# mbhall88/nohuman

Measured on AMD Instinct MI355X. Metric: Mreads/sec classified (HPRC.r2 DB, 150bp PE), higher is better.
Workload: dtype u64

## Files before the change

### nohuman_amd/csrc/nh_device.h

```cpp
#pragma once
#include <stdint.h>

namespace nh {

struct DevDB {
    const uint32_t *table;
    uint64_t copy_stride;
    uint32_t n_copies;
    uint32_t copy_shift;
    uint64_t capacity;
    uint64_t cap_magic;
    const uint32_t *parent;
    uint32_t node_count;
    uint32_t value_bits;
    uint32_t vmask;
    uint32_t k, l;
    uint32_t window;
    uint64_t lmer_mask;
    uint64_t spaced_mask;
    uint64_t toggle;
    uint64_t min_hash;
    int32_t revcom_version;
    int32_t linear_probing;
    int32_t reset_per_mate;
    uint32_t min_hit_groups;
    int32_t ambig_rule;
    uint32_t max_chunks;
};

enum { CNT_FRAGMENTS = 0, CNT_CLASSIFIED = 1, CNT_BASES = 2, CNT_LOOKUPS = 3, CNT_N = 4 };

struct Result {
    uint32_t call, total_kmers, clade_hits, hit_groups;
};

struct Sched {
    uint64_t n0, n01, total;
    uint64_t base1, base2;
    uint32_t c0, c1, c2, pad;
};

constexpr uint32_t TAIL_SHARDS = 8;
constexpr uint32_t WORK_WORDS = 1 + TAIL_SHARDS;
constexpr uint32_t WORK_STRIDE = 16;
constexpr uint32_t WORK_PASSES = 3;
constexpr uint32_t COUNTER_SHARDS = 64;
constexpr uint32_t COUNTER_STRIDE = 16;

constexpr uint32_t SEG_TILES = 32;
constexpr uint32_t SPLIT_MIN_TILES = 48;
constexpr uint32_t MID_TILES = 8;
constexpr uint32_t PART_DWORDS = 64;
constexpr uint32_t PART_CAP = 30;
struct SplitItem {
    uint32_t f, seg, nseg, slot;
};
struct SplitHdr {
    uint32_t n_multi, n_mid, n_small, seg_used;
};
struct SplitBufs {
    SplitHdr *hdr;
    SplitItem *items_multi;
    uint32_t *items_single;
    uint32_t *part;
    uint32_t *part_done;
    uint32_t seg_cap, pad;
};

struct KArgs {
    DevDB db;
    const uint8_t *bases;
    const uint64_t *seq_off;
    const uint32_t *seq_len;
    uint64_t bases_end;
    uint64_t n_frag;
    int32_t mates;
    uint32_t frag_chunk;
    Sched sched;
    double confidence;
    Result *out;
    uint32_t *kmer_taxa;
    const uint64_t *kmer_taxa_off;
    unsigned long long *counters;
    unsigned long long *cshard;
    int *error_flag;
    int *pending;
    uint32_t *defer_bits;
    int *pending_long;
    int32_t only_deferred;
    unsigned long long *work;
    SplitBufs split;
    unsigned long long *timeline;
};

struct SchedKnobs {
    bool set = false, off = false;
    uint32_t c1 = 0, c2 = 0, p1 = 100, p2 = 100;
};
struct LaunchIO {
    const void *d_bases = nullptr;
    const void *d_seq_off = nullptr;
    const void *d_seq_len = nullptr;
    uint64_t bases_end = 0;
    uint64_t n_frag = 0;
    int mates = 1;
    bool long_reads = false;
    void *d_out = nullptr, *d_kmer_taxa = nullptr;
    const void *d_kmer_taxa_off = nullptr;
    void *d_counters = nullptr;
};
struct LaunchSlot {
    int *d_error = nullptr;
    int *d_pending = nullptr;
    int *d_pending_long = nullptr;
    unsigned long long *d_work = nullptr;
    unsigned long long *d_cshard = nullptr;
    uint32_t *d_defer = nullptr;
    uint64_t defer_cap_bits = 0;
    SplitBufs split = {};
    uint64_t split_single_cap = 0;
    bool split_fresh = false;
};

constexpr uint32_t TAXON_AMBIGUOUS = 0xFFFFFFFFu;
constexpr uint32_t TAXON_MATE_BORDER = 0xFFFFFFFEu;

constexpr int WAVE = 64;
constexpr int WAVES_PER_BLOCK = 4;
constexpr int TL = 128;
constexpr int LIST_CAP = 64;

}
```

### nohuman_amd/csrc/nh_engine.hip

```cpp
#include <hip/hip_runtime.h>
#include <stdarg.h>
#include <stdio.h>
#include <stdlib.h>
#include <string.h>
#include <sys/stat.h>
#include <algorithm>
#include <thread>
#include <unistd.h>
#include <fcntl.h>

#include <chrono>
#include <mutex>
#include <string>
#include <vector>

#include "nh_device.h"
#include <map>

#include "nh_internal.h"
#include "nohuman_engine.h"

namespace nh {

namespace {
// ... 271 lines not shown
    d.node_count = (uint32_t)i.node_count;
    d.value_bits = (uint32_t)i.value_bits;
    d.vmask = (uint32_t)((1ull << i.value_bits) - 1);
    d.k = (uint32_t)i.k;
    d.l = (uint32_t)i.l;
    d.window = (uint32_t)(i.k - i.l);
    d.lmer_mask = (1ull << (2 * i.l)) - 1;
    d.spaced_mask = i.spaced_seed_mask ? i.spaced_seed_mask : ~0ull;
    d.toggle = i.toggle_mask & d.lmer_mask;
    d.min_hash = i.minimum_acceptable_hash_value;
    d.revcom_version = i.revcom_version;
    d.linear_probing = e->options.linear_probing;
    d.reset_per_mate = e->options.reset_per_mate;
    d.min_hit_groups = e->options.minimum_hit_groups;
    d.ambig_rule = e->options.ambiguity_rule == NH_AMBIGUITY_LAST_LMER ? 0 : 1;
    d.max_chunks = i.capacity + 1 > 0xFFFFFFFFull ? 0xFFFFFFFFu : (uint32_t)(i.capacity + 1);
}

void finish_devdb_public(Engine *e) { finish_devdb(e); }

static int alloc_table(Engine *e, uint64_t capacity) {
    e->table_cells_alloc = ((capacity + 3) & ~3ull) + 32;
    uint32_t want = 4;
    if (const char *env = getenv("NOHUMAN_TABLE_COPIES")) {
        const int v = atoi(env);
        want = v >= 8 ? 8u : v >= 4 ? 4u : v >= 2 ? 2u : 1u;
    }
    {
        const nh_db_info &i = e->info;
        const bool std_geom = i.k == 35 && i.l == 31 && i.revcom_version != 0 && i.minimum_acceptable_hash_value == 0;
        bool quad = std_geom && e->options.linear_probing != 0;
#ifdef NH_NO_QUAD
        quad = false;
#endif
        if (capacity >= 0xFFFFFF00ull && !quad) want = 1;
    }
    bool trimmed = false;
    for (;; want >>= 1) {
        const uint64_t sh = 32 / want;
        const uint64_t stride = ((e->table_cells_alloc + 32 + 31) & ~31ull) - (want > 1 ? sh : 0);
        const size_t bytes = (size_t)(stride * want + 64) * sizeof(uint32_t) + 256;
        hipError_t he = hipMalloc(&e->d_table_raw, bytes);
        if (he != hipSuccess && !trimmed) {
            (void)hipGetLastError();
            run_cache_trim();
            dev_cache_trim();
            (void)dev_set(e->device);
            trimmed = true;
            he = hipMalloc(&e->d_table_raw, bytes);
        }
        if (he == hipSuccess) {
            if (dev_debug()) dev_register(e->d_table_raw, bytes, e->device);
            e->d_table = (uint32_t *)(((uintptr_t)e->d_table_raw + 127) & ~(uintptr_t)127);
            e->n_copies = want;
            e->copy_stride = stride;
            if (getenv("NOHUMAN_TRACE"))
                fprintf(stderr, "[nohuman trace] hash table: %u staggered cop%s of %.2f GB\n", want, want == 1 ? "y" : "ies",
                        (double)e->table_cells_alloc * 4 / 1e9);
            return NH_OK;
        }
        (void)hipGetLastError();
        if (want == 1) return set_error(NH_EOOM, "cannot allocate the hash table (%zu bytes)", bytes);
    }
}

int refresh_table_copies(Engine *e) {
    HIP_TRY(dev_set(e->device));
    HIP_TRY(hipDeviceSynchronize());
    for (uint32_t j = 1; j < e->n_copies; j++)
        HIP_TRY(hipMemcpyAsync(e->d_table + j * e->copy_stride, e->d_table, e->table_cells_alloc * sizeof(uint32_t),
                               hipMemcpyDeviceToDevice, e->stream));
    HIP_TRY(hipStreamSynchronize(e->stream));
    return NH_OK;
}

LaunchKnobs read_launch_knobs() {
    LaunchKnobs kn;
    if (const char *env = getenv("NOHUMAN_FRAG_CHUNK")) kn.frag_chunk = (uint32_t)std::max(1, atoi(env));
    if (const char *env = getenv("NOHUMAN_SEG_CAP")) {
        const long v = atol(env);
        if (v >= 1) kn.seg_cap = (uint64_t)v;
    }
    kn.sched = parse_sched_knobs(getenv("NOHUMAN_SCHED"));
    return kn;
}

static int validate_table(Engine *e, bool check_size) {
    auto t0 = std::chrono::steady_clock::now();
    unsigned long long *d_out = (unsigned long long *)e->d_counters + CNT_N;
    unsigned long long out[2] = {0, 0};
    HIP_TRY(hipMemsetAsync(d_out, 0, sizeof out, e->stream));
    HIP_TRY(launch_validate_table(e->d_table, e->table_cells_alloc & ~3ull, (uint32_t)((1ull << e->info.value_bits) - 1), d_out, e->stream));
    HIP_TRY(hipMemcpyAsync(out, d_out, sizeof out, hipMemcpyDeviceToHost, e->stream));
    HIP_TRY(hipMemsetAsync(d_out, 0, sizeof out, e->stream));
    HIP_TRY(hipStreamSynchronize(e->stream));
    e->check.non_empty = out[0];
    e->check.max_value = out[1];
    e->check.seconds = std::chrono::duration<double>(std::chrono::steady_clock::now() - t0).count();
    if (getenv("NOHUMAN_TRACE"))
        fprintf(stderr, "[nohuman trace] hash table checked in %.4f s: %llu of %llu cells in use (load %.4f), largest value %llu, taxonomy nodes %llu\n",
                e->check.seconds, out[0], (unsigned long long)e->info.capacity, (double)out[0] / (double)e->info.capacity, out[1],
                (unsigned long long)e->info.node_count);
    if (out[1] >= e->info.node_count)
        return set_error(NH_EDB, "hash.k2d holds the taxon value %llu but taxo.k2d has only %llu nodes: the two files are not of one database",
                         out[1], (unsigned long long)e->info.node_count);
    if (check_size && out[0] != e->info.size)
        return set_error(NH_EDB, "hash.k2d: %llu cells are in use but its header says size %llu", out[0], (unsigned long long)e->info.size);
    return NH_OK;
}

static int common_open(Engine *e, int device) {
    int rc = check_device(device);
    if (rc) return rc;
    e->device = device;
    e->info.device = device;
    HIP_TRY(dev_set(device));
    hipDeviceProp_t prop;
    HIP_TRY(hipGetDeviceProperties(&prop, dev_phys(device)));
    e->n_cu = prop.multiProcessorCount;
    e->grid_blocks = e->n_cu * classify_blocks_per_cu();
    e->options.minimum_hit_groups = 2;
    e->options.linear_probing = 1;
    e->options.reset_per_mate = 1;
    e->options.ambiguity_rule = NH_AMBIGUITY_DEFAULT;
    bool overridden = false;
    if (const char *v = getenv("NOHUMAN_OPT_AMBIGUITY_RULE")) e->options.ambiguity_rule = atoi(v) != 0 ? NH_AMBIGUITY_QUEUE : NH_AMBIGUITY_LAST_LMER, overridden = true;
    if (const char *v = getenv("NOHUMAN_OPT_LINEAR_PROBING")) e->options.linear_probing = atoi(v) != 0, overridden = true;
    if (const char *v = getenv("NOHUMAN_OPT_RESET_PER_MATE")) e->options.reset_per_mate = atoi(v) != 0, overridden = true;
    if (const char *v = getenv("NOHUMAN_OPT_MIN_HIT_GROUPS")) e->options.minimum_hit_groups = (uint32_t)atoi(v), overridden = true;
    if (overridden) {
        static std::atomic<bool> said{false};
        if (!said.exchange(true))
            fprintf(stderr, "nohuman: WARN NOHUMAN_OPT_* overrides the classification switches of every engine of this process: ambiguity rule %s, "
                            "linear probing %d, per-mate reset %d, minimum hit groups %u\n",
                    e->options.ambiguity_rule == NH_AMBIGUITY_QUEUE ? "queue" : "last l-mer", e->options.linear_probing, e->options.reset_per_mate,
                    e->options.minimum_hit_groups);
    }
    e->knobs = read_launch_knobs();
    HIP_TRY(hipStreamCreateWithFlags(&e->stream, hipStreamNonBlocking));
    for (unsigned i = 0; i < LAUNCH_SLOTS; i++) HIP_TRY(hipEventCreateWithFlags(&e->slot_ev[i], hipEventDisableTiming));
    HIP_TRY(dev_malloc((void **)&e->d_counters, (CNT_N + 12) * sizeof(uint64_t)));
    HIP_TRY(hipMemset(e->d_counters, 0, (CNT_N + 12) * sizeof(uint64_t)));
    HIP_TRY(dev_malloc((void **)&e->d_work, LAUNCH_SLOTS * WORK_PASSES * WORK_WORDS * WORK_STRIDE * sizeof(unsigned long long)));
    HIP_TRY(hipMemset(e->d_work, 0, LAUNCH_SLOTS * WORK_PASSES * WORK_WORDS * WORK_STRIDE * sizeof(unsigned long long)));
    HIP_TRY(dev_malloc((void **)&e->d_cshard, LAUNCH_SLOTS * COUNTER_SHARDS * COUNTER_STRIDE * sizeof(unsigned long long)));
    HIP_TRY(hipMemset(e->d_cshard, 0, LAUNCH_SLOTS * COUNTER_SHARDS * COUNTER_STRIDE * sizeof(unsigned long long)));
    HIP_TRY(dev_malloc((void **)&e->d_error, (2 * LAUNCH_SLOTS + 1) * sizeof(int)));
    HIP_TRY(hipMemset(e->d_error, 0, (2 * LAUNCH_SLOTS + 1) * sizeof(int)));
    HIP_TRY(dev_malloc((void **)&e->d_defer, LAUNCH_SLOTS * DEFER_WORDS * sizeof(uint32_t)));
    HIP_TRY(hipMemset(e->d_defer, 0, LAUNCH_SLOTS * DEFER_WORDS * sizeof(uint32_t)));
    return NH_OK;
}

static int upload_taxonomy(Engine *e) {
    HIP_TRY(dev_malloc((void **)&e->d_parent, e->parent.size() * sizeof(uint32_t)));
    HIP_TRY(hipMemcpy(e->d_parent, e->parent.data(), e->parent.size() * sizeof(uint32_t),
                      hipMemcpyHostToDevice));
    return NH_OK;
}

void destroy(Engine *e) {
    if (!e) return;
    if (e->device >= 0) (void)dev_set(e->device);
    if (e->d_table_raw) (void)hipFree(e->d_table_raw);
    if (e->d_parent) (void)hipFree(e->d_parent);
    if (e->d_counters) (void)hipFree(e->d_counters);
    if (e->d_error) (void)hipFree(e->d_error);
    if (e->d_external) (void)hipFree(e->d_external);
    if (e->d_work) (void)hipFree(e->d_work);
    if (e->d_cshard) (void)hipFree(e->d_cshard);
    if (e->d_defer) (void)hipFree(e->d_defer);
    for (SplitBufs &sb : e->split)
        for (void *p : {(void *)sb.hdr, (void *)sb.items_multi, (void *)sb.items_single, (void *)sb.part, (void *)sb.part_done})
            if (p) (void)hipFree(p);
    for (void *p : {e->st.d_bases, e->st.d_offsets, e->st.d_results, e->st.d_taxa, e->st.d_taxa_off})
        if (p) (void)hipFree(p);
    for (hipEvent_t ev : e->slot_ev)
        if (ev) (void)hipEventDestroy(ev);
    if (e->stream) (void)hipStreamDestroy(e->stream);
    delete e;
}

int open_images(const void *opts, size_t opts_len, const void *taxo, size_t taxo_len,
                const void *hash, size_t hash_len, int device, Engine **out) {
    if (!opts || !taxo || !hash || !out) return set_error(NH_EINVAL, "null argument");
    Engine *e = new Engine();
    int rc = common_open(e, device);
    if (!rc) rc = parse_opts(e, opts, opts_len);
    if (!rc) rc = parse_taxonomy(e, taxo, taxo_len);
    if (!rc) {
        const uint8_t *hb = (const uint8_t *)hash;
        if (hash_len < 32) rc = set_error(NH_EDB, "hash.k2d: truncated header");
        else {
            e->info.capacity = rd64(hb);
            e->info.size = rd64(hb + 8);
            e->info.key_bits = rd64(hb + 16);
            e->info.value_bits = rd64(hb + 24);
            if (e->info.key_bits + e->info.value_bits != 32 || e->info.value_bits == 0 ||
                e->info.value_bits > 31)
                rc = set_error(NH_EDB, "hash.k2d: key_bits + value_bits != 32");
            else if (e->info.capacity == 0 || hash_len != 32 + 4 * e->info.capacity)
                rc = set_error(NH_EDB, "hash.k2d: size %zu != 32 + 4*capacity (%llu)", hash_len,
                               (unsigned long long)e->info.capacity);
        }
        if (!rc) rc = check_queue_packing(e);
        if (!rc) rc = alloc_table(e, e->info.capacity);
        if (!rc) {
            hipError_t he = hipMemset(e->d_table, 0, e->table_cells_alloc * sizeof(uint32_t));
            if (he == hipSuccess)
                he = hipMemcpy(e->d_table, hb + 32, 4 * e->info.capacity, hipMemcpyHostToDevice);
            if (he != hipSuccess) rc = set_error(NH_EDEVICE, "table upload: %s", hipGetErrorString(he));
        }
    }
    if (!rc) rc = validate_table(e, true);
    if (!rc) rc = upload_taxonomy(e);
    if (!rc) rc = refresh_table_copies(e);
    if (rc) {
        destroy(e);
        return rc;
    }
    finish_devdb(e);
// ... 692 lines not shown
```

### nohuman_amd/csrc/nh_internal.h

```cpp
#pragma once
#include <hip/hip_runtime.h>
#include <stdint.h>

#include <atomic>
#include <mutex>
#include <string>
#include <vector>

#include "nh_device.h"
#include "nohuman_engine.h"

namespace nh {
constexpr unsigned LAUNCH_SLOTS = 16;
constexpr uint64_t DEFER_WORDS = 1u << 15;
}

namespace nh {

struct Staging {
    void *d_bases = nullptr, *d_offsets = nullptr, *d_results = nullptr, *d_taxa = nullptr,
         *d_taxa_off = nullptr;
    size_t cap_bases = 0, cap_offsets = 0, cap_results = 0, cap_taxa = 0, cap_taxa_off = 0;
};

struct LaunchKnobs {
    uint32_t frag_chunk = 0;
    uint64_t seg_cap = 0;
    SchedKnobs sched;
};
LaunchKnobs read_launch_knobs();
SchedKnobs parse_sched_knobs(const char *env);

struct TableCheck {
    uint64_t non_empty = 0, max_value = 0;
    double seconds = 0;
};

struct Engine {
    int device = -1;
    int n_cu = 0;
    int grid_blocks = 0;
    nh_db_info info{};
    nh_options options{};
    DevDB dev{};
    void *d_table_raw = nullptr;
    uint32_t *d_table = nullptr;
    uint32_t n_copies = 1;
    uint64_t copy_stride = 0;
    uint64_t table_cells_alloc = 0;
    uint32_t *d_parent = nullptr;
    uint64_t *d_counters = nullptr;
    int *d_error = nullptr;
    unsigned long long *d_work = nullptr;
    unsigned long long *d_cshard = nullptr;
    uint32_t *d_defer = nullptr;
    SplitBufs split[LAUNCH_SLOTS] = {};
    uint64_t split_single_cap[LAUNCH_SLOTS] = {};
    bool split_fresh[LAUNCH_SLOTS] = {};
    std::mutex split_mu;
    std::atomic<unsigned> launch_seq{0};
    hipEvent_t slot_ev[LAUNCH_SLOTS] = {};
    bool slot_used[LAUNCH_SLOTS] = {};
    std::mutex slot_mu[LAUNCH_SLOTS];
    LaunchKnobs knobs;
    TableCheck check;
    hipStream_t stream = nullptr;
    std::vector<uint32_t> parent;
    std::vector<uint64_t> external;
    uint64_t *d_external = nullptr;
    std::vector<uint8_t> taxo_image, opts_image;
    Staging st;
    std::mutex mu;
    std::mutex db_mu;
    double seconds = 0;
};

extern thread_local std::string g_last_error;
int set_error(int code, const char *fmt, ...) __attribute__((format(printf, 2, 3)));

hipError_t launch_classify(const DevDB &db, const LaunchIO &io, double confidence, const LaunchSlot &sl,
                           uint32_t frag_chunk, int grid_blocks, hipStream_t stream, const SchedKnobs &sched_knobs);
Sched make_sched(uint64_t n_frag, uint32_t c0, int mates, uint64_t waves, const SchedKnobs &kn);
hipError_t launch_validate_table(const uint32_t *table, uint64_t n_cells, uint32_t vmask, unsigned long long *d_out2,
                                 hipStream_t stream);
int classify_blocks_per_cu();
hipError_t launch_insert_sequences(const DevDB &db, const void *d_bases, const void *d_seq_off,
                                   uint64_t n_seq, uint32_t value, unsigned long long *d_inserted,
                                   int grid_blocks, hipStream_t stream);
hipError_t launch_synth_insert(uint32_t *table, uint64_t capacity, uint64_t cap_magic,
                               uint32_t value_bits, uint32_t value, uint64_t n_keys, uint64_t seed,
                               uint64_t key_mask, unsigned long long *d_size, hipStream_t stream);

int open_dir(const char *db_dir, int device, Engine **out);
int open_images(const void *opts, size_t opts_len, const void *taxo, size_t taxo_len,
                const void *hash, size_t hash_len, int device, Engine **out);
int open_synthetic(uint64_t capacity, uint64_t n_keys, uint32_t depth, uint64_t seed, int device,
                   Engine **out);
void destroy(Engine *e);
void finish_devdb_public(Engine *e);
int refresh_table_copies(Engine *e);
int resolve_db_dir(const char *db_dir, std::string &resolved);
int classify_device(Engine *e, const void *d_bases, const void *d_seq_off, uint64_t n_frag,
                    uint32_t flags, double confidence, void *d_results, void *d_kmer_taxa,
                    const void *d_kmer_taxa_off, void *d_counters, hipStream_t stream,
                    const void *d_seq_len = nullptr, uint64_t bases_end = 0);
int classify_host(Engine *e, const uint8_t *bases, const uint64_t *seq_offsets, uint64_t n_frag,
                  uint32_t flags, double confidence, nh_result *results, uint32_t *kmer_taxa,
                  uint64_t *kmer_taxa_offsets, uint64_t kmer_taxa_cap);
int check_error_flag(Engine *e);
struct HumanOutArgs {
    const char *text;
// ... 64 lines not shown
```

### nohuman_amd/csrc/nh_kernels.hip

```cpp
#include <hip/hip_runtime.h>
#include <stdlib.h>
#include <string.h>

#include <type_traits>

#include "nh_device.h"

namespace nh {

#define NH_FULL 0xFFFFFFFFFFFFFFFFull
#ifndef NH_WIDE_CELLS
#define NH_WIDE_CELLS 16
#endif
#ifndef NH_WIDE_AFTER
#define NH_WIDE_AFTER 2
#endif
#ifndef NH_R2_CELLS
#define NH_R2_CELLS 4
#endif

template <bool STD> struct CandPad { static constexpr int value = STD ? 6 : 66; };

#ifndef NH_MIN_WAVES
#define NH_MIN_WAVES 5
// ... 1053 lines not shown
                                      kmer_taxa, kt, prof, tprev);
            if ((flags & 2u) && reset_per_mate) st.carry_tax = 0;
            bool finish = (flags & 1u) != 0;
            if (SPLIT && finish && (flags & 16u)) {
                const uint32_t nseg = uni(d0.y), seg = d_nk0, sb = uni(d1.w);
                KArgsP a4 = launder(ap);
                const bool over = st.overflow || st.nlist > PART_CAP;
                uint32_t v = 0;
                if (lane == 0) v = st.hit_groups;
                if (lane == 1) v = over ? 0u : st.nlist;
                if (lane == 2) v = over ? 1u : 0u;
                if (lane >= 4 && !over) {
                    const uint32_t idx = ((uint32_t)lane - 4u) >> 1;
                    if (idx < st.nlist) {
                        if constexpr (BIG) v = (lane & 1) ? TLI.cnt[idx] : TLI.tax[idx];
                        else v = (lane & 1) ? S.list_cnt[idx] : S.list_tax[idx];
                    }
                }
                __hip_atomic_store(&a4->split.part[(uint64_t)(sb + seg) * PART_DWORDS + (uint32_t)lane], v, __ATOMIC_RELAXED,
                                   __HIP_MEMORY_SCOPE_AGENT);
                asm volatile("s_waitcnt vmcnt(0)" ::: "memory");
                uint32_t old = 0;
                if (lane == 0) old = atomicAdd(&a4->split.part_done[sb], 1u);
                old = uni(old);
                finish = old + 1u == nseg;
                __atomic_signal_fence(__ATOMIC_SEQ_CST);
                if (finish) {
                    for (uint32_t s2 = 0; s2 < nseg; s2++) {
                        if (s2 == seg) continue;
                        const uint32_t pv = __hip_atomic_load(&a4->split.part[(uint64_t)(sb + s2) * PART_DWORDS + (uint32_t)lane],
                                                              __ATOMIC_RELAXED, __HIP_MEMORY_SCOPE_AGENT);
                        st.hit_groups += __builtin_amdgcn_readlane(pv, 0);
                        const uint32_t n2 = __builtin_amdgcn_readlane(pv, 1);
                        if (__builtin_amdgcn_readlane(pv, 2)) st.overflow = true;
                        for (uint32_t i = 0; i < n2; i++)
                            list_add<BIG>(S, TLI, lane, st, __builtin_amdgcn_readlane(pv, 4 + 2 * (int)i),
                                          __builtin_amdgcn_readlane(pv, 5 + 2 * (int)i));
                    }
                    if (over) st.overflow = true;
                }
            }
            if (finish) {
                const uint32_t total_kmers = d_total;
                uint32_t call = 0, clade_hits = 0;
                if (st.nlist > 0) {
                    if (BIG) {
                        call = resolve_tree_big(ap, TLI, lane, st, total_kmers, clade_hits);
                    } else if (st.nlist == 1) {
                        const uint32_t cnt = S.list_cnt[0];
                        const uint32_t required = (uint32_t)ceil(a2->confidence * (double)total_kmers);
                        call = cnt >= required ? S.list_tax[0] : 0u;
                        if (call && st.hit_groups < a2->db.min_hit_groups) call = 0;
                        clade_hits = call ? cnt : 0u;
                    } else {
                        call = resolve_tree<STD>(ap, S, lane, st, total_kmers, clade_hits);
                    }
                }
                const bool defer = !BIG && st.overflow;
                if (defer) call = 0;
                if (lane == 0) {
                    uint4 rec;
                    rec.x = defer ? CALL_OVERFLOW : call;
                    rec.y = total_kmers;
                    rec.z = clade_hits;
                    rec.w = st.hit_groups;
                    const uint32_t sn = S.stage_n;
                    S.stage_rec[sn] = rec;
                    S.stage_f[sn] = f;
                    S.stage_n = sn + 1;
                    if (kmer_taxa && mates == 2)
                        kmer_taxa[a2->kmer_taxa_off[f] + d_nk0] = TAXON_MATE_BORDER;
                    if (defer) atomicMax(&a2->pending[0], 1);
                    if (BIG && st.overflow) atomicOr(&a2->error_flag[0], 1);
                }
                if (lane == 0 && call) S.acc[CNT_CLASSIFIED] += 1;
            }
            wave_sync();
        }
        if (lane == 0) S.frag_state = make_uint4(st.nlist, st.hit_groups, st.carry_tax, st.overflow ? 1u : 0u);
        NH_STAMP(7);
    }

constexpr uint32_t PREF_LANES = 42;
constexpr uint32_t SHORT_MAX = 158;

__device__ __forceinline__ bool sample_all_long(KArgsP ap, const int lane) {
    KArgsP a = launder(ap);
    const uint64_t ns = a->n_frag * (uint64_t)a->mates;
    const uint64_t i = ns * (uint64_t)lane / 64u;
    const uint32_t len = a->seq_len != nullptr ? a->seq_len[i] : (uint32_t)(a->seq_off[i + 1] - a->seq_off[i]);
    return __ballot(len <= SHORT_MAX) == 0;
}

template <bool LINEAR, bool STD, bool CAP32, bool PROF, bool BIG>
__global__ __launch_bounds__(WAVE * WAVES_PER_BLOCK, BIG ? 1 : (STD ? NH_MIN_WAVES : 3)) void k_classify(const KArgs args_by_kernarg_pointer) {
    KArgsP ap = (KArgsP)__builtin_amdgcn_kernarg_segment_ptr();
    if (BIG && ap->pending[0] == 0) return;
    bool only_deferred = ap->only_deferred != 0;
    if (only_deferred && ap->pending_long[0] == 0) {
        if (BIG || !sample_all_long(ap, (int)(threadIdx.x & 63))) return;
        only_deferred = false;
    }
    typedef WaveLdsT<STD, 1, QCAP_GENERIC> WL;
    __shared__ WL lds_all[WAVES_PER_BLOCK];
    __shared__ uint32_t big_lists[BIG ? WAVES_PER_BLOCK * 3 * BIG_LIST_CAP : 1];
    const int lane = threadIdx.x & 63;
    const int wib = __builtin_amdgcn_readfirstlane(threadIdx.x >> 6);
    WL &S = lds_all[wib];
    TaxList TLI = {nullptr, nullptr, nullptr, 0};
    if constexpr (BIG) {
        TLI.tax = &big_lists[(wib * 3 + 0) * BIG_LIST_CAP];
        TLI.cnt = &big_lists[(wib * 3 + 1) * BIG_LIST_CAP];
        TLI.score = &big_lists[(wib * 3 + 2) * BIG_LIST_CAP];
        TLI.cap = BIG_LIST_CAP;
    }

    init_wave_lds<STD>(S, lane);

    const uint32_t K = STD ? 35u : ap->db.k;
    const uint32_t L = STD ? 31u : ap->db.l;
    const uint32_t TQ = TL - (STD ? 4u : ap->db.window);
    const int mates = ap->mates;
    const uint64_t n_frag = ap->n_frag;
    const bool reset_per_mate = ap->db.reset_per_mate != 0;
    const bool inplace = ap->seq_len != nullptr;
    if (lane == 0) S.last_dw = ((inplace ? ap->bases_end : ap->seq_off[n_frag * (uint64_t)mates]) + 4) >> 2;
    const uint32_t pl = (uint32_t)lane < PREF_LANES ? (uint32_t)lane : PREF_LANES - 1;

    auto tile_ptr = [&](uint64_t g0) -> const uint32_t * {
        KArgsP a3 = launder(ap);
        const uint64_t last_dw = S.last_dw;
        uint64_t dw = (g0 >> 2) + pl;
        dw = dw < last_dw ? dw : last_dw;
        return reinterpret_cast<const uint32_t *>(a3->bases) + dw;
    };

    if (lane < 4) S.acc[lane] = 0;
    bool bad_input = false;
    uint64_t prof[12] = {0, 0, 0, 0, 0, 0, 0, 0, 0, 0, 0, 0};
    uint64_t tprev = PROF ? __builtin_readcyclecounter() : 0;

#ifndef NH_PF_DEPTH
#define NH_PF_DEPTH 2
#endif
    constexpr int PFD = NH_PF_DEPTH;
    uint32_t tagf[PFD], wf[PFD];
#pragma unroll
    for (int i = 0; i < PFD; i++) tagf[i] = 0, wf[i] = 0;

    uint32_t par = 0;
    uint32_t nslot_new = 0;
    uint32_t nslot_old = 0;
    uint32_t qn = 0;
    LaneLookup lk;
    lk.busy = 0;
    lk.r = 0;
    lk.pos = lk.first_pos = lk.step = 0;
    lk.ckey = 0;
    lk.budget = 0;

    if (lane == 0) S.frag_state = make_uint4(0, 0, 0, 0);
    uint64_t carry_pack = 0;
    auto turn = [&]() {
        flush_records<STD>(ap, S, lane);
#ifndef NH_NO_QUAD
        if constexpr (LINEAR && STD)
// ... 202 lines not shown
                        d1.y = qn;
                        d1.z = nruns;
                        d1.w = seg_slot;
                        d2.x = (uint32_t)last_lane;
                        d2.y = (frag_end ? 1u : 0u) | (mate_end ? 2u : 0u) | (frag_first ? 4u : 0u) | (split ? 16u : 0u);
                        d2.z = split ? seg : nk0;
                        d2.w = nk0 + nk1;
                        if (split) d0.y = nseg;
                        uint4 *dp = reinterpret_cast<uint4 *>(&S.slot[par][nslot_new]);
                        dp[0] = d0;
                        dp[1] = d1;
                        dp[2] = d2;
                    }
                    S.ps[par][nslot_new][lane] = (uint16_t)ps;
                    NH_STAMP(10);
                    frag_first = false;
                    qn += nruns;
                    nslot_new++;
                    if (nslot_new == NSLOT || qn + TL > (uint32_t)QCAP_GENERIC) turn();
                }
            }
        }
    }
    turn();
    turn();
    flush_records<STD>(ap, S, lane);

    wave_sync();
    if (lane == 0) {
        unsigned long long *const counters = ap->counters;
        int *const error_flag = ap->error_flag;
        if (PROF && counters)
            for (int i = 0; i < 12; i++) atomicAdd(&counters[CNT_N + i], (unsigned long long)prof[i]);
        add_counters(ap, S.acc);
        if (bad_input) atomicOr(&error_flag[0], 2);
    }
}

template <bool PROF, bool WIDE, bool TLINE>
__global__ __launch_bounds__(WAVE * WAVES_PER_BLOCK, PROF ? 4 : NH_MIN_WAVES) void k_classify_short(const KArgs args_by_kernarg_pointer) {
    constexpr bool STD = true;
    KArgsP ap = (KArgsP)__builtin_amdgcn_kernarg_segment_ptr();
    typedef WaveLdsT<STD, NSLOT, QCAP_SHORT> WL;
    __shared__ WL lds_all[WAVES_PER_BLOCK];
    const int lane = threadIdx.x & 63;
    const int wib = __builtin_amdgcn_readfirstlane(threadIdx.x >> 6);
    WL &S = lds_all[wib];
    const TaxList TLI = {nullptr, nullptr, nullptr, 0};
    if (sample_all_long(ap, lane)) return;
    init_wave_lds<STD>(S, lane);

    constexpr uint32_t K = 35, L = 31;
    const int mates = ap->mates;
    const bool reset_per_mate = ap->db.reset_per_mate != 0;
    if (lane == 0)
        S.last_dw = ((ap->seq_len != nullptr ? ap->bases_end : ap->seq_off[ap->n_frag * (uint64_t)mates]) + 4) >> 2;
    const uint32_t pl = (uint32_t)lane < PREF_LANES ? (uint32_t)lane : PREF_LANES - 1;
    auto tile_ptr = [&](uint64_t g0) -> const uint32_t * {
        KArgsP a3 = launder(ap);
        const uint64_t last_dw = S.last_dw;
        uint64_t dw = (g0 >> 2) + pl;
        dw = dw < last_dw ? dw : last_dw;
        return reinterpret_cast<const uint32_t *>(a3->bases) + dw;
    };
    if (lane < 4) S.acc[lane] = 0;
    bool bad_input = false;
    uint64_t prof[12] = {0, 0, 0, 0, 0, 0, 0, 0, 0, 0, 0, 0};
    uint64_t tprev = PROF ? __builtin_readcyclecounter() : 0;

    uint32_t par = 0, nslot_new = 0, nslot_old = 0, qn = 0;
    LaneLookup lk;
    lk.busy = 0;
    lk.r = 0;
    lk.pos = lk.first_pos = lk.step = 0;
    lk.ckey = 0;
    lk.budget = 0;
    if (lane == 0) S.frag_state = make_uint4(0, 0, 0, 0);

    auto tl_row = [&]() -> unsigned long long * {
        if constexpr (!TLINE) return nullptr;
        unsigned long long *const base = launder(ap)->timeline;
        return base ? base + 32ull * ((uint64_t)blockIdx.x * WAVES_PER_BLOCK + (uint32_t)wib) : nullptr;
    };
    if (TLINE && lane == 0) {
        if (unsigned long long *const tline = tl_row()) {
            tline[0] = wall_clock64();
            tline[2] = tline[3] = tline[6] = 0;
            uint32_t xcc;
            asm volatile("s_getreg_b32 %0, hwreg(HW_REG_XCC_ID)" : "=s"(xcc));
            tline[7] = xcc;
        }
    }
    Draw dr;
    dr.raw = 0;
    dr.word = 0;
    bool first_claim = true;
    bool claim_ahead = true;
    auto take_claim = [&]() {
        draw_raw(ap, lane, dr);
        claim_ahead = true;
    };

    uint64_t cbeg = 0, cbase = 0;
    uint32_t nseq = 0, t = 0;
    uint32_t off_v = 0, len_v = 0;
    uint32_t w[NSLOT];
#pragma unroll
    for (int j = 0; j < NSLOT; j++) w[j] = 0;
    uint64_t carry_min = NH_FULL;
    uint32_t drain = 0;
    for (;;) {
        bool batch = true;
        if (t >= nseq) {
            NH_STAMP(8);
            uint64_t claim = ~0ull;
            if (first_claim) {
                claim = (uint64_t)blockIdx.x * WAVES_PER_BLOCK + (uint32_t)wib;
                first_claim = false;
            } else if (drain == 0) {
                claim = settle(ap, lane, dr, launder(ap)->sched.n0, launder(ap)->sched.total);
            }
            uint64_t c0 = 0;
            uint32_t ncf = 0;
            if (claim == ~0ull || !claim_range(ap, claim, launder(ap)->n_frag, c0, ncf)) {
                if (drain == 2) break;
                drain++;
                batch = false;
            } else {
                claim_ahead = false;
                if (TLINE && lane == 0) {
                    if (unsigned long long *const tline = tl_row()) {
                        tline[4] = wall_clock64();
                        if (tline[6] < 24) tline[8 + tline[6]] = (tline[4] << 8) | ncf;
                        tline[6] += 1;
                    }
                }
                cbeg = c0;
                const uint32_t ns = ncf * (uint32_t)mates;
                const bool inplace = launder(ap)->seq_len != nullptr;
                const uint32_t nof = inplace ? ns : ns + 1;
                const uint64_t sidx = cbeg * (uint64_t)mates + ((uint32_t)lane < nof ? (uint32_t)lane : nof - 1);
                const uint64_t off64 = launder(ap)->seq_off[sidx];
                cbase = readlane64(off64, 0);
                const uint64_t crel = off64 - cbase;
                if (__ballot((crel >> 32) != 0)) bad_input = true;
                off_v = (uint32_t)crel;
                len_v = inplace ? launder(ap)->seq_len[sidx] : (uint32_t)__shfl_down((int)off_v, 1, 64) - off_v;
                if ((uint32_t)lane >= ns) len_v = 0;
                if (__ballot(len_v > SHORT_MAX)) {
                    if (lane == 0) {
                        atomicOr(&launder(ap)->defer_bits[claim >> 5], 1u << (claim & 31));
                        if (__hip_atomic_load(launder(ap)->pending_long, __ATOMIC_RELAXED, __HIP_MEMORY_SCOPE_AGENT) == 0)
                            atomicMax(launder(ap)->pending_long, 1);
                    }
                    nseq = 0;
                    t = 0;
                    take_claim();
                    continue;
                }
                const uint32_t cb = wave_sum(len_v);
                if (lane == 0) {
                    S.acc[CNT_FRAGMENTS] += ncf;
                    S.acc[CNT_BASES] += cb;
                }
                nseq = ns;
                t = 0;
#pragma unroll
                for (int j = 0; j < NSLOT; j++)
                    if ((uint32_t)j < nseq) w[j] = *tile_ptr(cbase + __builtin_amdgcn_readlane(off_v, j));
            }
        }
        uint32_t ambmask = 0;
        if (batch) {
            NH_STAMP(0);
#pragma unroll
            for (int j = 0; j < NSLOT; j++) {
                const uint32_t i = t + (uint32_t)j;
                if (i < nseq) {
                    const uint32_t o = __builtin_amdgcn_readlane(off_v, i), n = __builtin_amdgcn_readlane(len_v, i);
                    const bool amb = encode_tile<STD>(S, lane, (uint32_t)j, w[j], (uint32_t)(cbase + o) & 3u, n);
                    ambmask |= (amb ? 1u : 0u) << j;
                }
                const uint32_t i2 = i + NSLOT;
                if (i2 < nseq) w[j] = *tile_ptr(cbase + __builtin_amdgcn_readlane(off_v, i2));
            }
            wave_sync();
            NH_STAMP(1);
            if (TLINE && lane == 0) {
                unsigned long long *const tline = tl_row();
                if (tline && tline[2] == 0) tline[2] = wall_clock64();
            }
            if (!claim_ahead && t + NSLOT >= nseq) take_claim();
        }
        for (uint32_t j = 0; j <= (uint32_t)NSLOT; j++) {
            const uint32_t i = t + j;
            if (batch && j < (uint32_t)NSLOT && i < nseq) {
                const uint32_t o = __builtin_amdgcn_readlane(off_v, i), n = __builtin_amdgcn_readlane(len_v, i);
                const uint32_t nk = n >= K ? n - K + 1 : 0;
                const uint32_t m = mates == 2 ? (i & 1u) : 0u;
                const uint64_t f = cbeg + (mates == 2 ? i >> 1 : i);
                uint32_t nk_other = 0;
                if (mates == 2) {
                    const uint32_t no = __builtin_amdgcn_readlane(len_v, i ^ 1u);
                    nk_other = no >= K ? no - K + 1 : 0;
                }
                const uint32_t nk0 = m ? nk_other : nk, nk1 = mates == 2 ? (m ? nk : nk_other) : 0u;
                if (nk0 + nk1 == 0) {
                    if (lane == 0 && m == (uint32_t)mates - 1) {
                        KArgsP a2 = launder(ap);
                        uint4 rec = {0, 0, 0, 0};
                        *reinterpret_cast<uint4 *>(&a2->out[f]) = rec;
                        uint32_t *const kmer_taxa = a2->kmer_taxa;
                        if (kmer_taxa && mates == 2) kmer_taxa[a2->kmer_taxa_off[f]] = TAXON_MATE_BORDER;
                    }
                } else if (nk != 0) {
                    if (m == 0 || nk0 == 0 || reset_per_mate) carry_min = NH_FULL;
                    const bool frag_first = m == 0 || nk0 == 0;
                    const bool frag_end = m == (uint32_t)mates - 1 || nk1 == 0;
                    const bool mate_end = m == 0 && mates == 2 && nk1 != 0;
                    uint32_t ps;
                    int last_lane;
                    const uint32_t nruns = scan_body<STD, PROF>(ap, S, lane, j, (ambmask >> j) & 1u,
                                                                (uint32_t)(cbase + o) & 3u, n - L + 1, nk, par, qn,
                                                                carry_min, ps, last_lane, prof, tprev);
                    if (lane == 0) {
                        uint4 d0, d1, d2;
                        d0.x = (uint32_t)f;
                        d0.y = (uint32_t)(f >> 32);
                        d0.z = m ? nk0 + 1 : 0;
                        d0.w = 0;
                        d1.x = nk;
                        d1.y = qn;
                        d1.z = nruns;
                        d1.w = 0;
                        d2.x = (uint32_t)last_lane;
                        d2.y = (frag_end ? 1u : 0u) | (mate_end ? 2u : 0u) | (frag_first ? 4u : 0u);
                        d2.z = nk0;
                        d2.w = nk0 + nk1;
                        uint4 *dp = reinterpret_cast<uint4 *>(&S.slot[par][nslot_new]);
                        dp[0] = d0;
                        dp[1] = d1;
                        dp[2] = d2;
                    }
                    S.ps[par][nslot_new][lane] = (uint16_t)ps;
                    NH_STAMP(10);
                    qn += nruns;
                    nslot_new++;
                }
            }
            const bool full = nslot_new == (uint32_t)NSLOT || qn + TL > (uint32_t)QCAP_SHORT;
            if ((nslot_new != 0 && (full || j == (uint32_t)NSLOT)) || (!batch && j == (uint32_t)NSLOT)) {
                flush_records<STD>(ap, S, lane);
#ifdef NH_NO_QUAD
                probe_queue<true, STD, !WIDE, PROF>(ap, S, lane, par, qn, lk, true, 0ull, prof, tprev);
#else
                probe_queue_quad<PROF, WIDE>(ap, S, lane, par, qn, lk, true, 0ull, prof, tprev);
#endif
                if (TLINE && lane == 0) {
                    unsigned long long *const tline = tl_row();
                    if (tline && tline[3] == 0) tline[3] = wall_clock64();
                }
                if (nslot_old)
                    post_group<STD, false, PROF, false>(ap, S, TLI, lane, mates, reset_per_mate, par ^ 1u, nslot_old, prof, tprev);
                nslot_old = nslot_new;
                par ^= 1u;
                nslot_new = 0;
                qn = 0;
            }
        }
        if (batch) t += NSLOT;
    }
    flush_records<STD>(ap, S, lane);

    wave_sync();
    if (lane == 0) {
        unsigned long long *const counters = ap->counters;
        int *const error_flag = ap->error_flag;
        if (PROF && counters)
            for (int i = 0; i < 12; i++) atomicAdd(&counters[CNT_N + i], (unsigned long long)prof[i]);
        add_counters(ap, S.acc);
        if (bad_input) atomicOr(&error_flag[0], 2);
        if constexpr (TLINE)
            if (unsigned long long *const tline = tl_row()) tline[5] = wall_clock64();
    }
}

struct FinishArgs {
    unsigned long long *cshard, *counters, *work;
    uint32_t *defer;
    uint32_t n_defer_words;
    int *pending_long, *pending;
    SplitHdr *split_hdr;
};
__global__ __launch_bounds__(64) void k_finish_launch(const FinishArgs a) {
    const int lane = threadIdx.x;
    unsigned long long v[4];
#pragma unroll
    for (int i = 0; i < 4; i++) {
        unsigned long long x = 0;
        for (uint32_t r = lane; r < COUNTER_SHARDS; r += 64) {
            x += a.cshard[(size_t)r * COUNTER_STRIDE + i];
            a.cshard[(size_t)r * COUNTER_STRIDE + i] = 0;
        }
        for (int d = 32; d >= 1; d >>= 1) x += __shfl_xor(x, d, 64);
        v[i] = x;
    }
    if (lane == 0 && a.counters)
        for (int i = 0; i < 4; i++)
            if (v[i]) atomicAdd(&a.counters[i], v[i]);
    if ((uint32_t)lane < WORK_PASSES * WORK_WORDS) a.work[(size_t)lane * WORK_STRIDE] = 0;
    for (uint32_t w = lane; w < a.n_defer_words; w += 64) a.defer[w] = 0;
    if (lane == 0) {
        *a.pending_long = 0;
        *a.pending = 0;
        if (a.split_hdr) *a.split_hdr = SplitHdr{0, 0, 0, 0};
    }
}

__device__ __forceinline__ uint32_t wave_scan_incl(uint32_t v, const int lane) {
#pragma unroll
    for (int d = 1; d < 64; d <<= 1) {
        const uint32_t o = (uint32_t)__shfl_up((int)v, d, 64);
        if (lane >= d) v += o;
    }
    return v;
}

__global__ __launch_bounds__(256) void k_prep_items(const KArgs args_by_kernarg_pointer) {
    KArgsP ap = (KArgsP)__builtin_amdgcn_kernarg_segment_ptr();
    const int lane = threadIdx.x & 63;
    const uint64_t n_frag = ap->n_frag;
    const uint64_t f = (uint64_t)blockIdx.x * blockDim.x + threadIdx.x;
    const bool act = f < n_frag;
    const uint32_t K = ap->db.k, TQ = TL - ap->db.window;
    uint64_t len = 0;
    if (act) len = ap->seq_len ? (uint64_t)ap->seq_len[f] : ap->seq_off[f + 1] - ap->seq_off[f];
    if (len > 0x7FFFFFFFull) len = 0x7FFFFFFFull;
    const uint32_t nk = len >= K ? (uint32_t)len - K + 1 : 0;
    const uint32_t nt = (nk + TQ - 1) / TQ;
    uint32_t nseg = nt > SPLIT_MIN_TILES ? (nt + SEG_TILES - 1) / SEG_TILES : 1u;
    bool multi = act && nseg > 1;
    SplitHdr *const hdr = ap->split.hdr;
    const uint32_t cap = ap->split.seg_cap;
    {
// ... 379 lines not shown
```

Measured before the change: 1033.

## Pipeline next-chunk claim, offset load and tile prefetch across batches

Replaces the boolean claim-ahead flag with a multi-stage state machine. The next chunk's claim is settled and its seq_off/seq_len loaded after a probe pass, and its first tiles are staged during the last batch of the current chunk, so dependent global loads overlap with hashing work instead of stalling at chunk boundaries. It also adds per-wave timeline event logging and a NOHUMAN_GRID_BLOCKS knob to cap the grid. The cost is more live state and registers per wave, and more complex drain and long-read defer logic.

```diff
diff --git a/nohuman_amd/csrc/nh_device.h b/nohuman_amd/csrc/nh_device.h
--- a/nohuman_amd/csrc/nh_device.h
+++ b/nohuman_amd/csrc/nh_device.h
@@ -92,6 +92,7 @@
     SplitBufs split;
     unsigned long long *timeline;
 };
+constexpr uint32_t TL_ROWS = 8192, TL_EVENTS = 512;
 
 struct SchedKnobs {
     bool set = false, off = false;
diff --git a/nohuman_amd/csrc/nh_engine.hip b/nohuman_amd/csrc/nh_engine.hip
--- a/nohuman_amd/csrc/nh_engine.hip
+++ b/nohuman_amd/csrc/nh_engine.hip
@@ -377,6 +377,7 @@
         if (v >= 1) kn.seg_cap = (uint64_t)v;
     }
     kn.sched = parse_sched_knobs(getenv("NOHUMAN_SCHED"));
+    if (const char *env = getenv("NOHUMAN_GRID_BLOCKS")) kn.grid_blocks = std::max(1, atoi(env));
     return kn;
 }
 
@@ -432,6 +433,7 @@
                     e->options.minimum_hit_groups);
     }
     e->knobs = read_launch_knobs();
+    if (e->knobs.grid_blocks && e->knobs.grid_blocks < e->grid_blocks) e->grid_blocks = e->knobs.grid_blocks;
     HIP_TRY(hipStreamCreateWithFlags(&e->stream, hipStreamNonBlocking));
     for (unsigned i = 0; i < LAUNCH_SLOTS; i++) HIP_TRY(hipEventCreateWithFlags(&e->slot_ev[i], hipEventDisableTiming));
     HIP_TRY(dev_malloc((void **)&e->d_counters, (CNT_N + 12) * sizeof(uint64_t)));
diff --git a/nohuman_amd/csrc/nh_internal.h b/nohuman_amd/csrc/nh_internal.h
--- a/nohuman_amd/csrc/nh_internal.h
+++ b/nohuman_amd/csrc/nh_internal.h
@@ -27,6 +27,7 @@
     uint32_t frag_chunk = 0;
     uint64_t seg_cap = 0;
     SchedKnobs sched;
+    int grid_blocks = 0;
 };
 LaunchKnobs read_launch_knobs();
 SchedKnobs parse_sched_knobs(const char *env);
diff --git a/nohuman_amd/csrc/nh_kernels.hip b/nohuman_amd/csrc/nh_kernels.hip
--- a/nohuman_amd/csrc/nh_kernels.hip
+++ b/nohuman_amd/csrc/nh_kernels.hip
@@ -1159,6 +1159,7 @@
     }
 
 constexpr uint32_t PREF_LANES = 42;
+constexpr uint32_t TLE_CHUNK = 1, TLE_BATCH = 2, TLE_FIRST = 16, TLE_LAST = 32;
 constexpr uint32_t SHORT_MAX = 158;
 
 __device__ __forceinline__ bool sample_all_long(KArgsP ap, const int lane) {
@@ -1527,6 +1528,18 @@
         unsigned long long *const base = launder(ap)->timeline;
         return base ? base + 32ull * ((uint64_t)blockIdx.x * WAVES_PER_BLOCK + (uint32_t)wib) : nullptr;
     };
+    uint32_t tl_nev = 0;
+    bool tl_batch_seen = false, tl_probe_seen = false;
+    uint32_t tl_nchunk = 0;
+    auto tl_event = [&](const uint32_t tag) {
+        if constexpr (TLINE) {
+            unsigned long long *const base = launder(ap)->timeline;
+            const uint64_t wv = (uint64_t)blockIdx.x * WAVES_PER_BLOCK + (uint32_t)wib;
+            if (lane == 0 && base && wv < TL_ROWS && tl_nev < TL_EVENTS)
+                base[32ull * TL_ROWS + wv * TL_EVENTS + tl_nev] = ((unsigned long long)wall_clock64() << 16) | tag;
+            tl_nev++;
+        }
+    };
     if (TLINE && lane == 0) {
         if (unsigned long long *const tline = tl_row()) {
             tline[0] = wall_clock64();
@@ -1539,11 +1552,11 @@
     Draw dr;
     dr.raw = 0;
     dr.word = 0;
-    bool first_claim = true;
-    bool claim_ahead = true;
+    enum : uint32_t { AHEAD_FIRST = 0, AHEAD_IDLE = 1, AHEAD_DRAWN = 2, AHEAD_OFFS = 3, AHEAD_TILES = 4, AHEAD_END = 5 };
+    uint32_t ahead = AHEAD_FIRST;
     auto take_claim = [&]() {
         draw_raw(ap, lane, dr);
-        claim_ahead = true;
+        ahead = AHEAD_DRAWN;
     };
 
     uint64_t cbeg = 0, cbase = 0;
@@ -1554,65 +1567,97 @@
     for (int j = 0; j < NSLOT; j++) w[j] = 0;
     uint64_t carry_min = NH_FULL;
     uint32_t drain = 0;
+
+    uint32_t claim_n_lo = 0, claim_n_hi = 0;
+    auto claim_n = [&]() -> uint64_t { return ((uint64_t)uni(claim_n_hi) << 32) | uni(claim_n_lo); };
+    uint64_t off64_n = 0;
+    uint32_t len_n = 0;
+    auto look_ahead = [&]() {
+        uint64_t claim;
+        if (ahead == AHEAD_FIRST)
+            claim = (uint64_t)blockIdx.x * WAVES_PER_BLOCK + (uint32_t)wib;
+        else
+            claim = settle(ap, lane, dr, launder(ap)->sched.n0, launder(ap)->sched.total);
+        uint64_t c0 = 0;
+        uint32_t ncf = 0;
+        if (claim == ~0ull || !claim_range(ap, claim, launder(ap)->n_frag, c0, ncf)) {
+            ahead = AHEAD_END;
+            return;
+        }
+        asm volatile("v_mov_b32 %0, %1" : "=v"(claim_n_lo) : "s"((uint32_t)claim));
+        asm volatile("v_mov_b32 %0, %1" : "=v"(claim_n_hi) : "s"((uint32_t)(claim >> 32)));
+        const uint32_t ns = ncf * (uint32_t)mates;
+        const bool inplace = launder(ap)->seq_len != nullptr;
+        const uint32_t nof = inplace ? ns : ns + 1;
+        const uint64_t sidx = c0 * (uint64_t)mates + ((uint32_t)lane < nof ? (uint32_t)lane : nof - 1);
+        off64_n = launder(ap)->seq_off[sidx];
+        if (inplace) len_n = launder(ap)->seq_len[sidx];
+        ahead = AHEAD_OFFS;
+    };
+    auto stage_ahead = [&]() {
+        uint64_t c0 = 0;
+        uint32_t ncf = 0;
+        const uint64_t claim = claim_n();
+        (void)claim_range(ap, claim, launder(ap)->n_frag, c0, ncf);
+        const uint32_t ns = ncf * (uint32_t)mates;
+        const uint64_t cbase_n = readlane64(off64_n, 0);
+        const uint64_t crel = off64_n - cbase_n;
+        if (__ballot((crel >> 32) != 0)) bad_input = true;
+        const uint32_t o32 = (uint32_t)crel;
+        if (launder(ap)->seq_len == nullptr) len_n = (uint32_t)__shfl_down((int)o32, 1, 64) - o32;
+        if ((uint32_t)lane >= ns) len_n = 0;
+        if (__ballot(len_n > SHORT_MAX)) {
+            if (lane == 0) {
+                atomicOr(&launder(ap)->defer_bits[claim >> 5], 1u << (claim & 31));
+                if (__hip_atomic_load(launder(ap)->pending_long, __ATOMIC_RELAXED, __HIP_MEMORY_SCOPE_AGENT) == 0)
+                    atomicMax(launder(ap)->pending_long, 1);
+            }
+            take_claim();
+            return;
+        }
+        const uint32_t cb = wave_sum(len_n);
+        if (lane == 0) {
+            S.acc[CNT_FRAGMENTS] += ncf;
+            S.acc[CNT_BASES] += cb;
+        }
+#pragma unroll
+        for (int j = 0; j < NSLOT; j++)
+            if ((uint32_t)j < ns) w[j] = *tile_ptr(cbase_n + __builtin_amdgcn_readlane(o32, j));
+        ahead = AHEAD_TILES;
+    };
     for (;;) {
         bool batch = true;
         if (t >= nseq) {
             NH_STAMP(8);
-            uint64_t claim = ~0ull;
-            if (first_claim) {
-                claim = (uint64_t)blockIdx.x * WAVES_PER_BLOCK + (uint32_t)wib;
-                first_claim = false;
-            } else if (drain == 0) {
-                claim = settle(ap, lane, dr, launder(ap)->sched.n0, launder(ap)->sched.total);
-            }
-            uint64_t c0 = 0;
-            uint32_t ncf = 0;
-            if (claim == ~0ull || !claim_range(ap, claim, launder(ap)->n_frag, c0, ncf)) {
+            tl_event(TLE_CHUNK);
+            if (ahead == AHEAD_FIRST || ahead == AHEAD_DRAWN) look_ahead();
+            if (ahead == AHEAD_OFFS) stage_ahead();
+            if (ahead == AHEAD_TILES) {
+                ahead = AHEAD_IDLE;
+                uint32_t ncf = 0;
+                (void)claim_range(ap, claim_n(), launder(ap)->n_frag, cbeg, ncf);
+                if (TLINE && lane == 0) {
+                    if (unsigned long long *const tline = tl_row()) {
+                        const unsigned long long now = wall_clock64();
+                        tline[4] = now;
+                        if (tl_nchunk < 24) tline[8 + tl_nchunk] = (now << 8) | ncf;
+                        tline[6] = tl_nchunk + 1;
+                    }
+                }
+                tl_nchunk++;
+                cbase = readlane64(off64_n, 0);
+                off_v = (uint32_t)(off64_n - cbase);
+                len_v = len_n;
+                nseq = ncf * (uint32_t)mates;
+                t = 0;
+            } else if (ahead == AHEAD_DRAWN) {
+                nseq = 0;
+                t = 0;
+                continue;
+            } else {
                 if (drain == 2) break;
                 drain++;
                 batch = false;
-            } else {
-                claim_ahead = false;
-                if (TLINE && lane == 0) {
-                    if (unsigned long long *const tline = tl_row()) {
-                        tline[4] = wall_clock64();
-                        if (tline[6] < 24) tline[8 + tline[6]] = (tline[4] << 8) | ncf;
-                        tline[6] += 1;
-                    }
-                }
-                cbeg = c0;
-                const uint32_t ns = ncf * (uint32_t)mates;
-                const bool inplace = launder(ap)->seq_len != nullptr;
-                const uint32_t nof = inplace ? ns : ns + 1;
-                const uint64_t sidx = cbeg * (uint64_t)mates + ((uint32_t)lane < nof ? (uint32_t)lane : nof - 1);
-                const uint64_t off64 = launder(ap)->seq_off[sidx];
-                cbase = readlane64(off64, 0);
-                const uint64_t crel = off64 - cbase;
-                if (__ballot((crel >> 32) != 0)) bad_input = true;
-                off_v = (uint32_t)crel;
-                len_v = inplace ? launder(ap)->seq_len[sidx] : (uint32_t)__shfl_down((int)off_v, 1, 64) - off_v;
-                if ((uint32_t)lane >= ns) len_v = 0;
-                if (__ballot(len_v > SHORT_MAX)) {
-                    if (lane == 0) {
-                        atomicOr(&launder(ap)->defer_bits[claim >> 5], 1u << (claim & 31));
-                        if (__hip_atomic_load(launder(ap)->pending_long, __ATOMIC_RELAXED, __HIP_MEMORY_SCOPE_AGENT) == 0)
-                            atomicMax(launder(ap)->pending_long, 1);
-                    }
-                    nseq = 0;
-                    t = 0;
-                    take_claim();
-                    continue;
-                }
-                const uint32_t cb = wave_sum(len_v);
-                if (lane == 0) {
-                    S.acc[CNT_FRAGMENTS] += ncf;
-                    S.acc[CNT_BASES] += cb;
-                }
-                nseq = ns;
-                t = 0;
-#pragma unroll
-                for (int j = 0; j < NSLOT; j++)
-                    if ((uint32_t)j < nseq) w[j] = *tile_ptr(cbase + __builtin_amdgcn_readlane(off_v, j));
             }
         }
         uint32_t ambmask = 0;
@@ -1631,11 +1676,13 @@
             }
             wave_sync();
             NH_STAMP(1);
-            if (TLINE && lane == 0) {
-                unsigned long long *const tline = tl_row();
-                if (tline && tline[2] == 0) tline[2] = wall_clock64();
-            }
-            if (!claim_ahead && t + NSLOT >= nseq) take_claim();
+            if (TLINE && lane == 0 && !tl_batch_seen) {
+                if (unsigned long long *const tline = tl_row()) tline[2] = wall_clock64();
+            }
+            tl_batch_seen = true;
+            tl_event(TLE_BATCH | (t == 0 ? TLE_FIRST : 0u) | (t + NSLOT >= nseq ? TLE_LAST : 0u) | (nseq << 8));
+            if (ahead == AHEAD_OFFS && t + NSLOT >= nseq) stage_ahead();
+            if (ahead == AHEAD_IDLE && t + 2 * NSLOT >= nseq) take_claim();
         }
         for (uint32_t j = 0; j <= (uint32_t)NSLOT; j++) {
             const uint32_t i = t + j;
@@ -1701,10 +1748,11 @@
 #else
                 probe_queue_quad<PROF, WIDE>(ap, S, lane, par, qn, lk, true, 0ull, prof, tprev);
 #endif
-                if (TLINE && lane == 0) {
-                    unsigned long long *const tline = tl_row();
-                    if (tline && tline[3] == 0) tline[3] = wall_clock64();
-                }
+                if (TLINE && lane == 0 && !tl_probe_seen) {
+                    if (unsigned long long *const tline = tl_row()) tline[3] = wall_clock64();
+                }
+                tl_probe_seen = true;
+                if (batch && ahead == AHEAD_DRAWN && t + NSLOT < nseq) look_ahead();
                 if (nslot_old)
                     post_group<STD, false, PROF, false>(ap, S, TLI, lane, mates, reset_per_mate, par ^ 1u, nslot_old, prof, tprev);
                 nslot_old = nslot_new;
```

Result: faster. 1070, median of 6 (+3.6%).
